# AntonXue/nn-sdp

Measured on NVIDIA B200. Metric: queries/sec (clique LMI blocks assembled: value * cliques_per_query), higher is better.
Workload: dtype f64

## Files before the change

### nn-sdp_b200/csrc/api.cu

```cuda
#include <math.h>
#include <stdarg.h>
#include <stdio.h>
#include <stdlib.h>
#include <string.h>

#include <algorithm>
#include <condition_variable>
#include <deque>
#include <functional>
#include <memory>
#include <mutex>
#include <thread>
#include <unordered_map>

#include <cuda.h>

#include "internal.h"

namespace nnsdp {

static thread_local std::string g_err;

void set_error(const char* fmt, ...) {
  char buf[1024];
// ... 748 lines not shown
  NN_TRY(b->xmax.ensure((size_t)sh.xtot * Q * 8));
  NN_TRY(b->acxmin.ensure((size_t)ac * Q * 8));
  NN_TRY(b->acxmax.ensure((size_t)ac * Q * 8));
  NN_TRY(b->smin_c.ensure((size_t)ac * Q * 8));
  NN_TRY(b->smax_c.ensure((size_t)ac * Q * 8));
  if (b->ring > 0) {
    const int npart = (int)((ac + PREP_THREADS - 1) / PREP_THREADS);
    NN_TRY(b->d11.ensure((size_t)ac * Q * 8));
    NN_TRY(b->Md.ensure((size_t)ac * Q * 8));
    NN_TRY(b->T0.ensure((size_t)ac * Q * 8));
    NN_TRY(b->Bt.ensure((size_t)ac * Q * 8 * std::max<int64_t>(beta, 1)));
    NN_TRY(b->u.ensure((size_t)ac * Q * 8));
    NN_TRY(b->aff.ensure((size_t)sh.Zdim * Q * 8));
    NN_TRY(b->part.ensure((size_t)npart * Q * 8));
    NN_TRY(b->act.ensure((size_t)ac * Q * 4));
    NN_TRY(b->cnt.ensure((size_t)sh.K * Q * 4));
    NN_TRY(b->Z11.ensure((size_t)sh.n_in() * sh.n_in() * Q * 8));
    NN_TRY(b->Z1K.ensure((size_t)sh.n_in() * sh.n[sh.K - 1] * Q * 8));
    NN_TRY(b->U.ensure((size_t)sh.n_out() * sh.n[sh.K - 1] * Q * 8));
    b->bd.npart = npart;
    const long long go = gram_layout(sh, &b->goff, &b->ldG);
    b->gram_per_query = go;
    NN_TRY(upload(b->d_goff, b->goff.data(), b->goff.size() * 8, b->st));
    NN_TRY(upload(b->d_ldG, b->ldG.data(), b->ldG.size() * 4, b->st));
    NN_TRY(b->gram.ensure((size_t)go * b->ring * 8));
    std::vector<CliqueRanges> mats;
    NN_TRY(format_mats(sh, beta, dense_Z, &mats));
    const char* noclass = getenv("NNSDP_NO_TILE_CLASSES");
    NN_TRY(build_plan(sh, beta, mats, b->packed || !(noclass && noclass[0] == '1'), &b->plan,
                      b->packed ? &b->lay : nullptr));
    b->mats_host = mats;
    for (const BandDev& j : b->plan.bands) b->band_max_m = std::max(b->band_max_m, j.m);
    b->nbands = (int)b->plan.bands.size();
    NN_TRY(upload(b->d_bands, b->plan.bands.data(), b->plan.bands.size() * sizeof(BandDev), b->st));
    if (!b->packed) NN_TRY(build_gather_plan(sh, beta, mats, b->plan, &b->gp));
    if (const char* e = getenv("NNSDP_DENSE_GATHER"))
      if (e[0] == '1') b->gp.usable = false;
    if (b->gp.usable) {
      NN_TRY(upload(b->d_thin_idx, b->gp.thin_idx.data(), b->gp.thin_idx.size() * 8, b->st));
      for (int i = 0; i < GATHER_STAGES; ++i)
        NN_CUDA(cudaEventCreateWithFlags(&b->ev_packed[i], cudaEventDisableTiming));
    }
    NN_TRY(upload(b->d_tiles, b->plan.tiles.data(), b->plan.tiles.size() * sizeof(TileDev), b->st));
    NN_TRY(upload(b->d_mats, b->plan.mats.data(), b->plan.mats.size() * sizeof(MatDev), b->st));
    NN_TRY(b->ringbuf.ensure((size_t)b->plan.per_query_doubles * b->ring * 8));
    b->slot_bulk.assign((size_t)b->ring * sh.K, 0);
    auto is_bulk = [&](const StripDev& d) {
      return !b->packed && d.rblk >= 1 && d.rblk <= sh.K - 1 &&
             (d.prog == PROG_SAME || (d.prog == PROG_DIAG && !b->plan.band_inline));
    };
    std::vector<StripDev> strips, bulk;
    std::vector<std::vector<StripDev>> per_blk(sh.K);
    b->pass_entries = 0;
    b->bulk_entries.assign(sh.K, 0);
    for (const StripDev& d : b->plan.strips) {
      if (d.prog == PROG_ZERO) continue;
      if (is_bulk(d)) {
        per_blk[d.rblk].push_back(d);
        b->bulk_entries[d.rblk] += (int64_t)d.nrows * d.ncols;
      } else {
        strips.push_back(d);
        b->pass_entries += (int64_t)d.nrows * d.ncols;
      }
    }
    b->bulk_begin.assign(sh.K + 1, 0);
    for (int blk = 0; blk < sh.K; ++blk) {
      b->bulk_begin[blk] = (int)bulk.size();
      bulk.insert(bulk.end(), per_blk[blk].begin(), per_blk[blk].end());
    }
    b->bulk_begin[sh.K] = (int)bulk.size();
    for (int i = b->plan.n_fill; i < (int)b->plan.tiles.size(); ++i)
      b->pass_entries += (int64_t)b->plan.tiles[i].nrows * b->plan.tiles[i].ncols;
    for (const BandDev& j : b->plan.bands)
      if (j.ld > 0) b->pass_entries += (int64_t)j.m * (2 * beta + 1) - beta * (beta + 1);
    NN_TRY(upload(b->d_strips, strips.data(), strips.size() * sizeof(StripDev), b->st));
    NN_TRY(upload(b->d_bulk, bulk.data(), bulk.size() * sizeof(StripDev), b->st));
    b->pd.strips = b->d_strips.as<StripDev>();
    b->pd.bulk = b->d_bulk.as<StripDev>();
    b->pd.n_strips = (int)strips.size();
    b->pd.tiles = b->d_tiles.as<TileDev>();
    b->pd.mats = b->d_mats.as<MatDev>();
    b->pd.panel_desc = nullptr;
    b->pd.n_panel = 0;
    {
      static const int panel_env = [] { const char* e = getenv("NNSDP_PANEL"); return e ? atoi(e) : 1; }();
      if (panel_env && !b->packed && !b->plan.panel.empty()) {
        std::vector<StripDev> panel;
        for (const StripDev& d : b->plan.panel)
          if (d.prog != PROG_ZERO && (d.prog == PROG_RC || d.prog == PROG_CR || !is_bulk(d))) panel.push_back(d);
        NN_TRY(upload(b->d_panel, panel.data(), panel.size() * sizeof(StripDev), b->st));
        b->pd.panel_desc = b->d_panel.as<StripDev>();
        b->pd.n_panel = (int)panel.size();
      }
    }
    b->pd.ntiles = (int)b->plan.tiles.size();
    b->pd.n_fill = b->plan.n_fill;
    b->pd.n_window = b->plan.n_window;
    b->pd.n_edge = b->plan.n_edge;
    b->pd.tile_rows = b->plan.tile_rows;
    b->pd.per_query = b->plan.per_query_doubles;
    b->pd.tmaps = nullptr;
    b->pd.tmap_ok = nullptr;
    if (b->plan.n_window > 0 && beta <= MAX_WINDOW_BETA) {
      typedef CUresult (*EncodeFn)(CUtensorMap*, CUtensorMapDataType, cuuint32_t, void*, const cuuint64_t*, const cuuint64_t*,
                                   const cuuint32_t*, const cuuint32_t*, CUtensorMapInterleave, CUtensorMapSwizzle,
                                   CUtensorMapL2promotion, CUtensorMapFloatOOBfill);
      void* fn = nullptr;
      cudaDriverEntryPointQueryResult qres;
      static const bool no_tma = [] { const char* e = getenv("NNSDP_NO_TMA"); return e && e[0] == '1'; }();
      if (!no_tma && cudaGetDriverEntryPoint("cuTensorMapEncodeTiled", &fn, cudaEnableDefault, &qres) == cudaSuccess && fn &&
          qres == cudaDriverEntryPointSuccess) {
        std::vector<CUtensorMap> maps(sh.K);
        std::vector<int> ok(sh.K, 0);
        bool any = false;
        for (int k = 0; k < sh.K; ++k) {
          if (sh.n[k + 1] % 2 != 0) continue;
          const cuuint64_t dims[2] = {(cuuint64_t)sh.n[k + 1], (cuuint64_t)sh.n[k]};
          const cuuint64_t strides[1] = {(cuuint64_t)sh.n[k + 1] * 8};
          const cuuint32_t box[2] = {(cuuint32_t)(128 + 2 * beta + 2), 32};
          const cuuint32_t estr[2] = {1, 1};
          const CUresult r = ((EncodeFn)fn)(&maps[k], CU_TENSOR_MAP_DATA_TYPE_FLOAT64, 2, b->nd->M[k].p, dims, strides, box, estr,
                                            CU_TENSOR_MAP_INTERLEAVE_NONE, CU_TENSOR_MAP_SWIZZLE_NONE,
                                            CU_TENSOR_MAP_L2_PROMOTION_L2_128B, CU_TENSOR_MAP_FLOAT_OOB_FILL_NONE);
          ok[k] = (r == CUDA_SUCCESS);
          any |= ok[k] != 0;
        }
        if (any) {
          static_assert(sizeof(CUtensorMap) == 128, "CUtensorMap is 128 bytes");
          NN_TRY(upload(b->d_tmaps, maps.data(), maps.size() * sizeof(CUtensorMap), b->st));
          NN_TRY(upload(b->d_tmap_ok, ok.data(), ok.size() * 4, b->st));
          NN_CUDA(cudaStreamSynchronize(b->st));
          b->pd.tmaps = b->d_tmaps.p;
          b->pd.tmap_ok = b->d_tmap_ok.as<int>();
        }
      } else {
        cudaGetLastError();
      }
    }
    b->pd.packed = b->plan.skip_absent ? 1 : 0;
    b->pd.band_inline = b->plan.band_inline ? 1 : 0;
    b->gd.scratch = b->gram.as<double>();
    b->gd.per_query = go;
    b->gd.goff = b->d_goff.as<long long>();
    b->gd.ldG = b->d_ldG.as<int>();
    b->gd.mirror = b->packed && b->plan.skip_absent ? 0 : 1;
  }
  NN_CUDA(cudaStreamSynchronize(b->st));
  guard.b = nullptr;
  *out = b;
  return NNSDP_OK;
}

int32_t nnsdp_batch_set_inputs(nnsdp_batch* b, int64_t Q, const nnsdp_query_inputs* in) {
  NN_CHECK(b && in, NNSDP_ERR_ARG, "NULL argument");
  NN_CHECK(Q >= 1 && Q <= b->Qcap, NNSDP_ERR_ARG, "Q = %lld outside [1, Qcap = %lld]", (long long)Q,
           (long long)b->Qcap);
  NN_CUDA(cudaSetDevice(b->dev));
  const Shape& sh = b->net->sh;
  const nnsdp_sizes& sz = b->sz;
  BatchDev& bd = b->bd;
  cudaStream_t st = b->st;
  b->have_inputs = false;
  b->bounds_done = b->prepared = false;
  b->Q = Q;
  bd.Q = (int)Q;
  bd.beta = (int)b->beta;
  bd.lamdim = sz.lamdim;
  bd.sdim = (int)sz.sdim;
  NN_TRY(upload_cols(b->x1min, in->x1min, in->x1min_stride, sz.n_in, Q, st, &bd.s_x1min, "x1min"));
  NN_TRY(upload_cols(b->x1max, in->x1max, in->x1max_stride, sz.n_in, Q, st, &bd.s_x1max, "x1max"));
  bd.x1min = b->x1min.as<double>();
  bd.x1max = b->x1max.as<double>();
  b->bounds_supplied = (in->ymin != nullptr);
  if (b->bounds_supplied) {
    NN_TRY(upload_cols(b->ymin, in->ymin, in->ymin_stride, sz.acdim, Q, st, &bd.s_ymin, "ymin"));
// ... 1721 lines not shown
```

### nn-sdp_b200/csrc/internal.h

```cpp
#pragma once

#include <cuda_runtime.h>
#include <stdint.h>

#include <string>
#include <vector>

#include "../../include/nnsdp_b200.h"

namespace nnsdp {

void set_error(const char* fmt, ...);
int32_t cuda_fail(cudaError_t e, const char* what, const char* file, int line);

#define NN_CUDA(call)                                                                \
  do {                                                                               \
    cudaError_t _e = (call);                                                         \
    if (_e != cudaSuccess) return ::nnsdp::cuda_fail(_e, #call, __FILE__, __LINE__); \
  } while (0)

#define NN_CHECK(cond, code, ...)      \
  do {                                 \
    if (!(cond)) {                     \
      ::nnsdp::set_error(__VA_ARGS__); \
// ... 41 lines not shown
int32_t make_cliques_host(const Shape& sh, int64_t beta, CliqueInfoHost* out);
int64_t lambda_dim(int64_t acdim, int64_t beta);
long long gram_layout(const Shape& sh, std::vector<long long>* goff, std::vector<int>* ldG);
int32_t fill_sizes(const Shape& sh, int64_t beta, nnsdp_sizes* out);

enum TileFlags : uint32_t {
  TF_AFF = 1u << 0,
  TF_SAME = 1u << 1,
  TF_1K = 1u << 2,
  TF_RC = 1u << 3,
  TF_CR = 1u << 4,
  TF_BAND = 1u << 5,
  TF_ALL = 0x3Fu,
  TF_UNIFORM = 1u << 8,
};

enum TileProg : int32_t {
  PROG_ZERO = 0, PROG_SAME = 1, PROG_RC = 2, PROG_CR = 3, PROG_MIXED = 4, PROG_GENERAL = 5,
  PROG_DIAG = 6, PROG_AFF = 7,
};

struct TileDev {
  int32_t mat;
  int32_t row0, nrows;
  int32_t col0, ncols;
  int32_t grow0;
  int32_t gcol0;
  uint32_t flags;
  int32_t rblk, cblk;
  int32_t prog;
};

struct alignas(16) StripDev {
  long long out_off;
  long long goff;
  int32_t ld, row0, nrows, col0;
  int32_t ncols, grow0, gcol0, prog;
  int32_t rblk, rl0, cl0, ldG;
};
static_assert(sizeof(StripDev) == 64, "StripDev must be 64 bytes");

struct MatDev {
  int64_t out_off;
  int32_t n;
  int32_t ld;
};

enum PackedKind : int32_t { PK_WINDOW = 1, PK_DIAG = 2, PK_BAND = 3, PK_RECT = 4 };
struct PackedCell {
  int32_t kind, blk;
  int64_t grow0, gcol0;
  int64_t nrows, ncols;
  int64_t offset;
  int32_t always;
};
struct PackedLayout {
  std::vector<PackedCell> cells;
  int64_t record_doubles = 0;
  int64_t always_doubles = 0;
  int64_t always_entries = 0;
  std::vector<int32_t> diag_cell;
  std::vector<int64_t> diag_entries;
};
struct BandDev {
  long long out_off;
  long long band_off;
  int ld, row0, col0;
  int g0, m, blk;
  int optional;
  int upper_only;
};

struct PlanHost {
  std::vector<StripDev> strips;
  std::vector<TileDev> tiles;
  std::vector<MatDev> mats;
  int64_t per_query_doubles = 0;
  int tile_rows = 0, tile_cols = 0;
  std::vector<BandDev> bands;
  bool band_inline = true;
  int n_fill = 0, n_window = 0, n_edge = 0;
  bool skip_absent = false;
  std::vector<StripDev> panel;
};

enum GatherKind : int32_t { GK_NONE = 0, GK_ALWAYS = 1, GK_GRAM = 2, GK_S22 = 3 };
constexpr int GATHER_MIN_RECT = 256;

struct GatherCell {
  int32_t row0, nrows;
  int32_t kind, blk;
  int32_t pure_zero;
  int32_t ncols_hint, col0_hint;
};
struct GatherColSeg {
  int32_t mat, col0, ncols;
  std::vector<GatherCell> cells;
};
struct GatherPlan {
  bool usable = false;
  std::vector<GatherColSeg> colsegs;
  std::vector<int32_t> colseg_begin;
  std::vector<int64_t> thin_idx;
  std::vector<int64_t> thin_begin;
  int64_t dense_always_doubles = 0;
};

int32_t build_plan(const Shape& sh, int64_t beta, const std::vector<CliqueRanges>& mats,
                   bool classify, PlanHost* plan, PackedLayout* packed = nullptr);
void unpack_record(const Shape& sh, int64_t beta, const PackedLayout& lay, const std::vector<CliqueRanges>& mats,
                   const double* record, const uint8_t* present, double* out);
int32_t build_gather_plan(const Shape& sh, int64_t beta, const std::vector<CliqueRanges>& mats,
                          const PlanHost& plan, GatherPlan* gp);

struct NetDev {
  int K, n_in, n_out, Zdim, acdim, xtot;
  const int* n;
  const int* off;
  const int* xoff;
  const int* blk_of;
  const double* const* M;
  const double* const* Wt;
  const int* ldT;
  const double* bias_all;
};

struct BatchDev {
  int Q, beta;
  int out_kind, has_s22, has_s12;
  int sdim;
  long long lamdim;
  const double* x1min;   long long s_x1min;
  const double* x1max;   long long s_x1max;
  const double* ymin;    long long s_ymin;
  const double* ymax;    long long s_ymax;
  const double* smin;    long long s_smin;
  const double* smax;    long long s_smax;
  const double* gin;     long long s_gin;
  const double* gbnd;    long long s_gbnd;
  const double* gsec;    long long s_gsec;
  const double* outS;    long long s_outS;
  const double* outvec;  long long s_outvec;
  const double* outinvP; long long s_outinvP;
  const double* gout;    long long s_gout;
  double* d11;
  double* Md;
  double* T0;
  double* Bt;
  double* u;
  double* aff;
  double* part;
  int npart;
  int* act;
  int* cnt;
  double* Z11;
  double* Z1K;
  double* U;
};

struct GramDev {
  double* scratch;
  long long per_query;
  const long long* goff;
  const int* ldG;
  int mirror;
};

struct PlanDev {
  const StripDev* strips;
  const StripDev* bulk;
  int n_strips;
  const TileDev* tiles;
  const MatDev* mats;
  const StripDev* panel_desc;
  int n_panel;
  int ntiles;
  int n_fill, n_window, n_edge;
  int tile_rows;
  long long per_query;
  const void* tmaps;
  const int* tmap_ok;
  int packed;
  int band_inline;
};

int ibp_layer_launch(const double* Mk, int n_out_k, int n_in_k, const double* xin_min,
                     const double* xin_max, long long x_stride, double* xout_min, double* xout_max,
                     double* acx_min, double* acx_max, long long acx_stride, int Q, int relu,
                     int write_x, int* flag_bad, cudaStream_t st);
int affine_layer_launch(const double* Wt, int ldT, int n_rows, int n_neurons, const double* u,
                        long long u_stride, double* aff, long long aff_stride, int Q,
                        cudaStream_t st);
int affine_all_launch(const NetDev& nd, int K, int max_rows, const double* u, long long u_stride, double* aff,
                      long long aff_stride, int Q, cudaStream_t st);
int ibp_all_launch(const NetDev& nd, int max_out, const double* x1min, long long s_min, const double* x1max,
                   long long s_max, double* xmin, double* xmax, long long x_stride, double* acxmin, double* acxmax,
                   double* smin, double* smax, long long acx_stride, int Q, int* flag_bad, cudaStream_t st);
int dgemm_dmma_launch(const double* A, int lda, int M, int K, const double* B, long long ldb, double* C, long long ldc,
                      int N, int accumulate, cudaStream_t st);
int ibp_dmma_launch(const double* Mk, int n_out_k, int n_in_k, const double* xin_min, const double* xin_max,
                    long long x_stride, double* xout_min, double* xout_max, double* acx_min, double* acx_max,
                    long long acx_stride, int Q, int relu, int write_x, int* flag_bad, cudaStream_t st);
int dgemm_dmma_affine_layers_launch(const NetDev& nd, int b0, int nb, int max_rows, const double* u, long long u_stride,
                                    double* aff, long long aff_stride, int Q, cudaStream_t st);
int ibp_chain_launch(const NetDev& nd, int max_w, const double* x1min, long long s_min, const double* x1max,
                     long long s_max, double* xmin, double* xmax, long long x_stride, double* acxmin, double* acxmax,
                     double* smin, double* smax, long long acx_stride, int Q, int* flag_bad, cudaStream_t st);
int launch_sector_minmax(long long n, const double* acxmin, const double* acxmax, double* smin,
                         double* smax, cudaStream_t st);
int launch_place_x1(const double* x1min, long long s_min, const double* x1max, long long s_max,
                    double* xmin, double* xmax, long long xtot, int n_in, int Q, cudaStream_t st);
int launch_transpose_w(const double* Mk, int n_out_k, int n_in_k, double* Wt, int ldT,
                       cudaStream_t st);
int launch_prep(const NetDev& net, const BatchDev& b, int* err_flag, cudaStream_t st);
int launch_gram(const NetDev& net, const BatchDev& b, const GramDev& g, int max_n, int q0, const int* pairs,
                int npairs, cudaStream_t st);
struct BulkItem {
  int32_t slot, first, count;
};
constexpr int BULK_PER_LAUNCH = 512;
struct BulkSel {
  int32_t n;
  BulkItem item[BULK_PER_LAUNCH];
};
int launch_emit(const NetDev& net, const BatchDev& b, const GramDev& g, const PlanDev& plan,
                int q0, int nq, double* out, cudaStream_t st, int which, const BulkItem* sel, int nsel);

struct AffineDev {
  long long nvar, var_out, var_bnd, var_sec;
  long long acdim, lamdim, beta;
  int out_kind;
  const double *x1min, *x1max, *ymin, *ymax, *smin, *smax;
  long long s_x1min, s_x1max, s_ymin, s_ymax, s_smin, s_smax;
  const long long* col_ptr;
  const int* lo;
};
int launch_affine_count(const NetDev& net, const AffineDev& A, long long* counts, cudaStream_t st);
int launch_affine_fill(const NetDev& net, const AffineDev& A, const long long* offs, long long* ent,
                       long long* var, double* val, cudaStream_t st);
int launch_affine_z0(const NetDev& net, const BatchDev& b, const AffineDev& A, long long nent, int Q, double* z0,
                     cudaStream_t st);
int launch_affine_csc_count(const NetDev& net, const AffineDev& A, const long long* first, long long ngroups,
                            long long* counts, cudaStream_t st);
int launch_affine_csc_fill(const NetDev& net, const AffineDev& A, const long long* first, long long ngroups,
                           const long long* offs, long long* ent, double* val, cudaStream_t st);
long long scan_scratch_len(long long n);
int launch_scan_exclusive(long long* x, long long n, long long* sums, cudaStream_t st);
int launch_affine_group_starts(const long long* offs, long long nvar, long long ngroups, long long* starts,
                               cudaStream_t st);

int launch_eig_init(double* v, int Zdim, int Qc, int q_first, cudaStream_t st);
int launch_eig_mid(const NetDev& net, const BatchDev& b, int q_first, int Qc, const double* x,
                   const double* t, double* s1, double* y, cudaStream_t st);
int launch_eig_io(const NetDev& net, const BatchDev& b, int q_first, int Qc, const double* x, double* y,
                  cudaStream_t st);
int launch_eig_multidot(const double* V, const double* w, int n, int Qc, int nv, double* c, int c_ld,
                        cudaStream_t st);
int launch_eig_project(const double* V, double* w, int n, int Qc, int nv, const double* c, int c_ld,
// ... 47 lines not shown
```

### nn-sdp_b200/csrc/kernels_emit.cu

```cuda
#include <stdlib.h>

#include <algorithm>

#include "internal.h"

namespace nnsdp {

namespace {

constexpr int ETHREADS = 256;
constexpr int SLOT_GROUP = 8;
constexpr int FAST_TR = 128, FAST_TC = 32, FAST_NCOL = 16;
constexpr int MAX_TAPS = 2 * MAX_FAST_BETA + 1;
constexpr int MAX_TC = 32;

struct QView {
  const double* Md;
  const double* T0;
  const double* Bt;
  const double* gbnd;
  const double* aff;
  const double* Z11;
  const double* Z1K;
  const double* U;
// ... 427 lines not shown
  const bool copy = Br <= K - 2 && b.cnt[(long long)q * K + Br] > 0;
  const bool s22 = Br == K - 1 && b.has_s22;
  if (plan.packed && !copy && !s22) return;
  const double* WK = net.M[K - 1];
  const double* U = b.U + (long long)q * net.n_out * net.n[K - 1];
  const double* G = g.scratch + (long long)slot * g.per_query + goff + rl0;
  if (BAND_INLINE && prog == PROG_DIAG) {
    const int beta = b.beta;
    const long long acdim = net.acdim;
    const int jr_base = grow0 - net.n_in - row0, jc0 = gcol0 - net.n_in;
    const double* T0 = b.T0 + (long long)q * acdim;
    const double* Bt = b.Bt + (long long)q * beta * acdim;
    const double* gbnd = b.gbnd + q * b.s_gbnd;
    const double* Gc = G + (long long)(cl0 + cg) * ldG;
    const long long gstep = (long long)ncg * ldG;
    for (int c = cg; c < ncols; c += ncg, col += cstep, Gc += gstep) {
      const int jc = jc0 + c;
      int r = row0 - (int)(((size_t)(col + row0) >> 3) & 3) + tr;
      for (; r < row_end; r += TR) {
        if (r < row0) continue;
        double v = copy ? Gc[r] : (s22 ? s22_entry(WK, U, net.n_out, rl0 + r, cl0 + c) : 0.0);
        const int d = jr_base + r - jc;
        if (d >= -beta && d <= beta) {
          v = 0.0 + v;
          v += 0.0;
          v = __dadd_rn(v, band_term(T0, gbnd, Bt, acdim, jc + d, jc));
        }
        col[r] = v;
      }
    }
  } else if (copy) {
    const double* Gc = G + (long long)(cl0 + cg) * ldG;
    const long long gstep = (long long)ncg * ldG;
    for (int c = cg; c < ncols; c += ncg, col += cstep, Gc += gstep) {
      int r = row0 - (int)(((size_t)(col + row0) >> 3) & 3) + tr;
      if (r >= row0 && r < row_end) col[r] = Gc[r];
      for (r += TR; r < row_end; r += TR) col[r] = Gc[r];
    }
  } else if (s22) {
    NNSDP_STRIP_LOOP(s22_entry(WK, U, net.n_out, rl0 + r, cl0 + c))
  } else {
    NNSDP_STRIP_LOOP(0.0)
  }
#undef NNSDP_STRIP_LOOP
}

template <bool BAND_INLINE>
__global__ void __launch_bounds__(ETHREADS, NNSDP_FILL_MINB)
emit_fill_kernel(NetDev net, BatchDev b, GramDev g, PlanDev plan, int q0, int nq,
                 double* __restrict__ out) {
  fill_strip<BAND_INLINE>(net, b, g, plan, plan.strips + blockIdx.x, blockIdx.y, q0, out);
}

template <bool BAND_INLINE>
__global__ void __launch_bounds__(ETHREADS, NNSDP_FILL_MINB)
emit_fill_kernel(NetDev net, BatchDev b, GramDev g, PlanDev plan, int q0, BulkSel sel, double* __restrict__ out) {
  const BulkItem it = sel.item[blockIdx.y];
  if ((int)blockIdx.x >= it.count) return;
  fill_strip<BAND_INLINE>(net, b, g, plan, plan.bulk + it.first + blockIdx.x, it.slot, q0, out);
}

template <int BETA>
__global__ void __launch_bounds__(ETHREADS, 4)
emit_window_kernel(NetDev net, BatchDev b, PlanDev plan, int tile0, int q0, int nq, int group, int group_major,
                   double* __restrict__ out) {
  constexpr int RC_DOUBLES = SLOT_GROUP * (BETA + 1) * (FAST_TC + BETA + 1), CR_DOUBLES = FAST_TC * CR_LDW(BETA);
  __shared__ __align__(128) double smem[RC_DOUBLES > CR_DOUBLES ? RC_DOUBLES : CR_DOUBLES];
  __shared__ __align__(8) unsigned long long mbar;
  const int ngroups = (nq + group - 1) / group;
  const int ti = group_major ? blockIdx.x % plan.n_window : blockIdx.x / ngroups;
  const int gi = group_major ? blockIdx.x / plan.n_window : blockIdx.x % ngroups;
  const TileDev t = plan.tiles[tile0 + ti];
  const MatDev mat = plan.mats[t.mat];
  const int slot0 = gi * group;
  const int nslots = min(group, nq - slot0);
  if (t.prog == PROG_RC) {
    if (t.ncols == FAST_TC) emit_rc<BETA, true>(net, b, plan, t, mat, q0, slot0, nslots, out, smem);
    else emit_rc<BETA, false>(net, b, plan, t, mat, q0, slot0, nslots, out, smem);
  } else {
    emit_cr<BETA>(net, b, plan, t, mat, q0, slot0, nslots, out, smem, &mbar);
  }
}

template <int BETA>
__global__ void __launch_bounds__(ETHREADS, 4)
emit_panel_kernel(NetDev net, BatchDev b, GramDev g, PlanDev plan, int q0, int nq, int group, double* __restrict__ out) {
  constexpr int RC_DOUBLES = SLOT_GROUP * (BETA + 1) * (FAST_TC + BETA + 1), CR_DOUBLES = FAST_TC * CR_LDW(BETA);
  __shared__ __align__(128) double smem[RC_DOUBLES > CR_DOUBLES ? RC_DOUBLES : CR_DOUBLES];
  __shared__ __align__(8) unsigned long long mbar;
  const int batch = group >> 8;
  group &= 255;
  const int gb = batch / group;
  const int per_batch = plan.n_panel * gb;
  const int sb = blockIdx.x / per_batch, rem = blockIdx.x - sb * per_batch;
  const int slot_lo = sb * batch, slot_hi = min(nq, slot_lo + batch);
  const int item = rem / gb, g0 = rem - item * gb;
  const StripDev* desc = plan.panel_desc + item;
  const int4* dp = reinterpret_cast<const int4*>(desc);
  const int4 d2 = __ldg(dp + 2);
  if (d2.w != PROG_RC && d2.w != PROG_CR) {
    for (int slot = slot_lo + g0; slot < slot_hi; slot += gb) fill_strip<false>(net, b, g, plan, desc, slot, q0, out);
    return;
  }
  const int4 d0 = __ldg(dp), d1 = __ldg(dp + 1), d3 = __ldg(dp + 3);
  TileDev t;
  t.mat = 0;
  t.row0 = d1.y, t.nrows = d1.z, t.col0 = d1.w, t.ncols = d2.x, t.grow0 = d2.y, t.gcol0 = d2.z, t.prog = d2.w;
  t.rblk = d3.x, t.cblk = d3.y, t.flags = (uint32_t)d3.z;
  MatDev mat;
  mat.out_off = ((long long)(unsigned)d0.x) | ((long long)d0.y << 32);
  mat.ld = d1.x;
  mat.n = d3.w;
  const int slot0 = slot_lo + g0 * group;
  const int nslots = min(group, slot_hi - slot0);
  if (nslots <= 0) return;
  if (t.prog == PROG_RC) {
    if (t.ncols == FAST_TC) emit_rc<BETA, true>(net, b, plan, t, mat, q0, slot0, nslots, out, smem);
    else emit_rc<BETA, false>(net, b, plan, t, mat, q0, slot0, nslots, out, smem);
  } else {
    emit_cr<BETA>(net, b, plan, t, mat, q0, slot0, nslots, out, smem, &mbar);
  }
}

__global__ void __launch_bounds__(ETHREADS, 4)
emit_edge_kernel(NetDev net, BatchDev b, GramDev g, PlanDev plan, int tile0, int q0, int nq,
                 int group, double* __restrict__ out) {
  __shared__ double smem[MAX_TC * MAX_TAPS + 128 * MAX_TAPS];
  const TileDev t = plan.tiles[tile0 + blockIdx.x];
  const MatDev mat = plan.mats[t.mat];
  const int slot0 = blockIdx.y * group;
  const int nslots = min(group, nq - slot0);
  int TR = 1;
  while (TR < t.nrows) TR <<= 1;
  if (TR > ETHREADS) TR = ETHREADS;
  const int tr = threadIdx.x % TR, cg = threadIdx.x / TR, ncg = ETHREADS / TR;
  const long long tile_off = mat.out_off + (t.row0 + tr) + (long long)t.col0 * mat.ld;
  const bool uniform = (t.flags & TF_UNIFORM) != 0 && t.nrows * t.ncols > 512;
  if (uniform) {
    for (int s = 0; s < nslots; ++s) {
      const QView v = make_view(net, b, g, q0 + slot0 + s, slot0 + s);
      double* o = out + (long long)(slot0 + s) * plan.per_query + tile_off;
      emit_mixed(net, b, g, t, mat, v, o, tr, cg, ncg, smem);
    }
    return;
  }
  int TC = 1;
  while (TC < t.ncols && TC < ncg) TC <<= 1;
  const int per = TR * TC;
  const int spar = ETHREADS / per;
  const int sub = threadIdx.x / per, cg2 = (threadIdx.x % per) / TR;
  for (int s = sub; s < nslots; s += spar) {
    const QView v = make_view(net, b, g, q0 + slot0 + s, slot0 + s);
    double* o = out + (long long)(slot0 + s) * plan.per_query + tile_off;
    emit_general(net, b, g, t, mat, v, o, tr, cg2, TC);
  }
}

}

namespace {
__device__ __forceinline__ void band_entry(const NetDev& net, const BatchDev& b, const GramDev& g, const BandDev& bd,
                                           long long per_query, int q0, int slot, int idx, double* __restrict__ out) {
  const int q = q0 + slot, K = net.K, beta = b.beta, nt = 2 * beta + 1;
  if (idx >= bd.m * nt) return;
  const int i = idx / nt, t = idx - i * nt - beta, c = i + t;
  if (bd.upper_only && t < 0) return;
  double* o = out + (long long)slot * per_query;
  if (c < 0 || c >= bd.m) {
    if (bd.band_off >= 0 && t >= 0) o[bd.band_off + t + (long long)(beta + 1) * i] = 0.0;
    return;
  }
  const int Br = bd.blk, n0 = net.n_in;
  const long long acdim = net.acdim;
  const int rl = bd.g0 - net.off[Br] + i, cl = rl + t;
  const int jr = bd.g0 + i - n0, jc = jr + t;
  const bool copy = Br <= K - 2 && b.cnt[(long long)q * K + Br] > 0;
  const bool s22 = Br == K - 1 && b.has_s22;
  double val = 0.0;
  if (copy) val += g.scratch[(long long)slot * g.per_query + g.goff[Br] + rl + (long long)cl * g.ldG[Br]];
  if (s22) val += s22_entry(net.M[K - 1], b.U + (long long)q * net.n_out * net.n[K - 1], net.n_out, rl, cl);
  val += 0.0;
  val = __dadd_rn(val, band_term(b.T0 + (long long)q * acdim, b.gbnd + q * b.s_gbnd, b.Bt + (long long)q * beta * acdim,
                                 acdim, jr, jc));
  if (bd.ld > 0 && (!bd.optional || copy || s22)) o[bd.out_off + (bd.row0 + i) + (long long)(bd.col0 + c) * bd.ld] = val;
  if (bd.band_off >= 0 && t >= 0) o[bd.band_off + t + (long long)(beta + 1) * i] = val;
}

__global__ void __launch_bounds__(ETHREADS)
emit_band_kernel(NetDev net, BatchDev b, GramDev g, const BandDev* __restrict__ bands, long long per_query, int q0,
                 int nq, int spc, double* __restrict__ out) {
  const BandDev bd = bands[blockIdx.y];
  const int idx = blockIdx.x * ETHREADS + threadIdx.x;
  for (int slot = blockIdx.z * spc; slot < min(nq, (blockIdx.z + 1) * spc); ++slot)
    band_entry(net, b, g, bd, per_query, q0, slot, idx, out);
}
}

int launch_emit_band(const NetDev& net, const BatchDev& b, const GramDev& g, const BandDev* bands, int nbands,
                     int max_m, long long per_query, int q0, int nq, double* out, cudaStream_t st) {
  if (nbands <= 0 || nq <= 0 || max_m <= 0) return 0;
  const int nx = (max_m * (2 * b.beta + 1) + ETHREADS - 1) / ETHREADS;
  static const int spc_env = [] { const char* e = getenv("NNSDP_BAND_GROUP"); return e ? atoi(e) : 0; }();
  const int spc = spc_env > 0 ? spc_env : (nq >= 16 ? 4 : 1);
  emit_band_kernel<<<dim3(nx, nbands, (nq + spc - 1) / spc), ETHREADS, 0, st>>>(net, b, g, bands, per_query, q0, nq, spc, out);
  return 1;
}

namespace {
__global__ void pack_thin_kernel(const double* __restrict__ ring, long long per_query,
                                 const long long* __restrict__ idx, long long nthin,
                                 double* __restrict__ packed, int nq) {
  const long long total = nthin * nq;
  for (long long i = blockIdx.x * (long long)blockDim.x + threadIdx.x; i < total;
       i += (long long)gridDim.x * blockDim.x) {
    const long long s = i / nthin, k = i - s * nthin;
    packed[i] = ring[s * per_query + idx[k]];
  }
}
}

int launch_pack_thin(const double* ring, long long per_query, const long long* idx, long long nthin,
                     double* packed, int nq, cudaStream_t st) {
  if (nthin <= 0 || nq <= 0) return 0;
  long long blocks = (nthin * nq + 255) / 256;
  if (blocks > 148 * 16) blocks = 148 * 16;
  pack_thin_kernel<<<(int)blocks, 256, 0, st>>>(ring, per_query, idx, nthin, packed, nq);
  return 1;
}

static int launch_bulk(const NetDev& net, const BatchDev& b, const GramDev& g, const PlanDev& plan, int q0,
                       const BulkItem* sel, int nsel, double* out, cudaStream_t st) {
  int launches = 0;
  for (int i0 = 0; i0 < nsel; i0 += BULK_PER_LAUNCH) {
    BulkSel s;
    s.n = std::min(BULK_PER_LAUNCH, nsel - i0);
    int most = 0;
    for (int i = 0; i < s.n; ++i) {
      s.item[i] = sel[i0 + i];
      most = std::max(most, s.item[i].count);
    }
    if (most == 0) continue;
    const dim3 grid((unsigned)most, (unsigned)s.n);
    if (plan.band_inline) emit_fill_kernel<true><<<grid, ETHREADS, 0, st>>>(net, b, g, plan, q0, s, out);
    else emit_fill_kernel<false><<<grid, ETHREADS, 0, st>>>(net, b, g, plan, q0, s, out);
    ++launches;
  }
  return launches;
}

int launch_emit(const NetDev& net, const BatchDev& b, const GramDev& g, const PlanDev& plan,
                int q0, int nq, double* out, cudaStream_t st, int which, const BulkItem* sel, int nsel) {
  if (nq <= 0) return 0;
  static const int wgroup = [] { const char* e = getenv("NNSDP_WINDOW_GROUP"); int v = e ? atoi(e) : 4; return v < 1 ? 1 : (v > SLOT_GROUP ? SLOT_GROUP : v); }();
  static const int egroup_env = [] { const char* e = getenv("NNSDP_EDGE_GROUP"); int v = e ? atoi(e) : 0; return v < 0 ? 0 : (v > SLOT_GROUP ? SLOT_GROUP : v); }();
  const int egroup = egroup_env > 0 ? egroup_env : (nq >= 64 ? SLOT_GROUP : (nq >= 16 ? 4 : 1));
  int launches = 0;
  if (plan.n_panel > 0 && b.beta <= MAX_WINDOW_BETA) {
    if (which < 0 || which == 0) {
      static const int pgroup = [] { const char* e = getenv("NNSDP_PANEL_GROUP"); int v = e ? atoi(e) : 2; return v < 1 ? 1 : (v > SLOT_GROUP ? SLOT_GROUP : v); }();
      static const int pbatch_env = [] { const char* e = getenv("NNSDP_PANEL_BATCH"); return e ? atoi(e) : 8; }();
      int pbatch = std::max(pgroup, (pbatch_env / pgroup) * pgroup);
      if (pbatch > 255) pbatch = (255 / pgroup) * pgroup;
      const int nbatches = (nq + pbatch - 1) / pbatch;
      const dim3 grid((unsigned)plan.n_panel * (pbatch / pgroup) * nbatches);
      switch (b.beta) {
        case 0: emit_panel_kernel<0><<<grid, ETHREADS, 0, st>>>(net, b, g, plan, q0, nq, pgroup | (pbatch << 8), out); break;
        case 1: emit_panel_kernel<1><<<grid, ETHREADS, 0, st>>>(net, b, g, plan, q0, nq, pgroup | (pbatch << 8), out); break;
        case 2: emit_panel_kernel<2><<<grid, ETHREADS, 0, st>>>(net, b, g, plan, q0, nq, pgroup | (pbatch << 8), out); break;
        case 3: emit_panel_kernel<3><<<grid, ETHREADS, 0, st>>>(net, b, g, plan, q0, nq, pgroup | (pbatch << 8), out); break;
        default: emit_panel_kernel<4><<<grid, ETHREADS, 0, st>>>(net, b, g, plan, q0, nq, pgroup | (pbatch << 8), out); break;
      }
      ++launches;
    }
  } else {
  if (plan.n_strips > 0 && (which < 0 || which == 0)) {
    if (plan.band_inline) emit_fill_kernel<true><<<dim3(plan.n_strips, nq), ETHREADS, 0, st>>>(net, b, g, plan, q0, nq, out);
    else emit_fill_kernel<false><<<dim3(plan.n_strips, nq), ETHREADS, 0, st>>>(net, b, g, plan, q0, nq, out);
    ++launches;
  }
  if (plan.n_window > 0 && (which < 0 || which == 1)) {
    const dim3 grid(plan.n_window * ((nq + wgroup - 1) / wgroup));
    const int t0 = plan.n_fill;
    static const int gm_env = [] { const char* e = getenv("NNSDP_WINDOW_GROUP_MAJOR"); return e ? atoi(e) : -1; }();
    const int gm = gm_env >= 0 ? gm_env : plan.band_inline;
    switch (b.beta) {
      case 0: emit_window_kernel<0><<<grid, ETHREADS, 0, st>>>(net, b, plan, t0, q0, nq, wgroup, gm, out); break;
      case 1: emit_window_kernel<1><<<grid, ETHREADS, 0, st>>>(net, b, plan, t0, q0, nq, wgroup, gm, out); break;
      case 2: emit_window_kernel<2><<<grid, ETHREADS, 0, st>>>(net, b, plan, t0, q0, nq, wgroup, gm, out); break;
      case 3: emit_window_kernel<3><<<grid, ETHREADS, 0, st>>>(net, b, plan, t0, q0, nq, wgroup, gm, out); break;
      case 4: emit_window_kernel<4><<<grid, ETHREADS, 0, st>>>(net, b, plan, t0, q0, nq, wgroup, gm, out); break;
      default: return -1;
    }
    ++launches;
  }
  }
  if (which < 0 || which == 0) launches += launch_bulk(net, b, g, plan, q0, sel, nsel, out, st);
  if (plan.n_edge > 0 && (which < 0 || which == 2)) {
    emit_edge_kernel<<<dim3(plan.n_edge, (nq + egroup - 1) / egroup), ETHREADS, 0, st>>>(
        net, b, g, plan, plan.n_fill + plan.n_window, q0, nq, egroup, out);
    ++launches;
  }
  return launches;
}

}
```

### nn-sdp_b200/csrc/plan.cpp

```cpp
#include <stdint.h>
#include <stdlib.h>

#include <algorithm>

#include "internal.h"
#include <atomic>
#include <cstring>
#include <thread>

namespace nnsdp {

int64_t lambda_dim(int64_t acdim, int64_t beta) {
  int64_t s = 0;
  for (int64_t t = acdim - beta; t <= acdim; ++t) s += t;
  return s;
}

long long gram_layout(const Shape& sh, std::vector<long long>* goff, std::vector<int>* ldG) {
  goff->assign(sh.K, 0);
  ldG->assign(sh.K, 0);
  long long go = 0;
  for (int blk = 0; blk <= sh.K - 2; ++blk) {
    (*ldG)[blk] = (int)(((sh.n[blk] + 15) / 16) * 16);
    (*goff)[blk] = go;
// ... 487 lines not shown
      }
      NN_CHECK(cell >= 0, NNSDP_ERR_STATE, "packed plan: a tile lies in no cell");
      const PackedCell& c = L.cells[cell];
      t.mat = cell;
      t.row0 = (int32_t)(t.grow0 - c.grow0);
      t.col0 = (int32_t)(t.gcol0 - c.gcol0);
      if (c.kind == PK_DIAG) L.diag_entries[c.blk] += (int64_t)t.nrows * t.ncols;
      else L.always_entries += (int64_t)t.nrows * t.ncols;
    }
    for (const PackedCell& c : band) L.always_entries += c.nrows * c.ncols;
    plan->per_query_doubles = L.record_doubles;
  }
  std::stable_sort(plan->tiles.begin(), plan->tiles.end(),
                   [&](const TileDev& x, const TileDev& y) { return cls(x) < cls(y); });
  {
    std::vector<long long> goff;
    std::vector<int> ldG;
    gram_layout(sh, &goff, &ldG);
    plan->strips.clear();
    for (const TileDev& t : plan->tiles) {
      if (cls(t) != 0) break;
      StripDev d{};
      d.out_off = plan->mats[t.mat].out_off;
      d.ld = plan->mats[t.mat].ld;
      d.row0 = t.row0; d.nrows = t.nrows; d.col0 = t.col0; d.ncols = t.ncols;
      d.grow0 = t.grow0; d.gcol0 = t.gcol0; d.prog = t.prog; d.rblk = t.rblk;
      if ((t.prog == PROG_SAME || t.prog == PROG_DIAG) && t.rblk >= 0) {
        d.rl0 = (int32_t)(t.grow0 - sh.off[t.rblk] - t.row0);
        d.cl0 = (int32_t)(t.gcol0 - sh.off[t.rblk]);
        if (t.rblk <= K - 2) {
          d.goff = goff[t.rblk];
          d.ldG = ldG[t.rblk];
        }
      }
      plan->strips.push_back(d);
    }
  }
  {
    plan->bands.clear();
    struct Box { int64_t lo = INT64_MAX, hi = -1, l0 = 0; bool band = false; };
    std::vector<std::vector<Box>> box(plan->mats.size(), std::vector<Box>(K));
    int64_t widest = 0;
    for (const TileDev& t : plan->tiles) {
      if (cls(t) != 0 || !(t.prog == PROG_SAME || t.prog == PROG_DIAG) || t.rblk < 1 || t.rblk != t.cblk) continue;
      Box& bx = box[t.mat][t.rblk];
      const int64_t lo = std::min<int64_t>(t.grow0, t.gcol0);
      if (lo < bx.lo) {
        bx.lo = lo;
        bx.l0 = (t.grow0 <= t.gcol0) ? t.row0 : t.col0;
      }
      bx.hi = std::max<int64_t>(bx.hi, std::max<int64_t>(t.grow0 + t.nrows, t.gcol0 + t.ncols) - 1);
      bx.band |= (t.prog == PROG_DIAG);
      widest = std::max<int64_t>(widest, bx.hi - bx.lo + 1);
    }
    plan->band_inline = widest < 256;
    for (size_t m = 0; m < plan->mats.size(); ++m)
      for (int blk = 1; blk < K; ++blk) {
        const Box& bx = box[m][blk];
        if (bx.hi < bx.lo || !bx.band) continue;
        BandDev j{};
        j.out_off = plan->mats[m].out_off;
        j.band_off = -1;
        j.ld = plan->band_inline ? 0 : plan->mats[m].ld;
        j.row0 = j.col0 = (int)bx.l0;
        j.g0 = (int)bx.lo;
        j.m = (int)(bx.hi - bx.lo + 1);
        j.blk = blk;
        if (packed) {
          const PackedCell& c = packed->cells[m];
          j.optional = (c.kind == PK_DIAG);
          j.upper_only = 1;
          for (const PackedCell& bc : packed->cells)
            if (bc.kind == PK_BAND && bc.blk == blk) j.band_off = bc.offset;
        }
        if (j.ld > 0 || j.band_off >= 0) plan->bands.push_back(j);
      }
  }
  plan->n_fill = plan->n_window = plan->n_edge = 0;
  for (const TileDev& t : plan->tiles) {
    const int c = cls(t);
    (c == 0 ? plan->n_fill : c == 1 ? plan->n_window : plan->n_edge)++;
  }
  plan->panel.clear();
  if (!packed && !plan->band_inline && plan->n_window > 0 && beta <= MAX_WINDOW_BETA) {
    struct Key { long long off; int panel, row0, col0, code; };
    std::vector<Key> keys;
    keys.reserve((size_t)plan->n_fill + plan->n_window);
    for (int i = 0; i < plan->n_fill; ++i) {
      const StripDev& d = plan->strips[i];
      keys.push_back({d.out_off, d.col0 / 32, d.row0, d.col0, i});
    }
    for (int i = 0; i < plan->n_window; ++i) {
      const TileDev& t = plan->tiles[plan->n_fill + i];
      keys.push_back({plan->mats[t.mat].out_off, t.col0 / 32, t.row0, t.col0, ~i});
    }
    std::stable_sort(keys.begin(), keys.end(), [](const Key& x, const Key& y) {
      if (x.off != y.off) return x.off < y.off;
      if (x.panel != y.panel) return x.panel < y.panel;
      if (x.col0 != y.col0) return x.col0 < y.col0;
      return x.row0 < y.row0;
    });
    plan->panel.resize(keys.size());
    for (size_t i = 0; i < keys.size(); ++i) {
      const int code = keys[i].code;
      if (code >= 0) {
        plan->panel[i] = plan->strips[code];
        continue;
      }
      const TileDev& t = plan->tiles[plan->n_fill + ~code];
      const MatDev& m = plan->mats[t.mat];
      StripDev d{};
      d.out_off = m.out_off;
      d.ld = m.ld;
      d.row0 = t.row0; d.nrows = t.nrows; d.col0 = t.col0; d.ncols = t.ncols;
      d.grow0 = t.grow0; d.gcol0 = t.gcol0; d.prog = t.prog;
      d.rblk = t.rblk; d.rl0 = t.cblk; d.cl0 = (int32_t)t.flags; d.ldG = m.n;
      plan->panel[i] = d;
    }
  }
  return NNSDP_OK;
}


static void unpack_one(int64_t beta, const PackedLayout& lay, const CliqueRanges& ck, const double* record,
                       const uint8_t* present, double* o) {
  const int64_t n = ck.size();
  std::memset(o, 0, (size_t)n * n * sizeof(double));
  constexpr int64_t TB = 64;
  auto copy_rect = [&](const PackedCell& c) {
    const double* src = record + c.offset;
    int64_t rbase = 0;
    for (int sr = 0; sr < ck.nseg; rbase += ck.hi[sr] - ck.lo[sr] + 1, ++sr) {
      const int64_t r0 = std::max(c.grow0, ck.lo[sr]), r1 = std::min(c.grow0 + c.nrows - 1, ck.hi[sr]);
      if (r0 > r1) continue;
      int64_t cbase = 0;
      for (int sc = 0; sc < ck.nseg; cbase += ck.hi[sc] - ck.lo[sc] + 1, ++sc) {
        const int64_t c0 = std::max(c.gcol0, ck.lo[sc]), c1 = std::min(c.gcol0 + c.ncols - 1, ck.hi[sc]);
        if (c0 > c1 || r0 > c1) continue;
        const int64_t lr_of = rbase - ck.lo[sr], lc_of = cbase - ck.lo[sc];
        for (int64_t gcb = std::max(c0, r0); gcb <= c1; gcb += TB) {
          const int64_t gce = std::min(gcb + TB - 1, c1);
          for (int64_t grb = r0; grb <= std::min(r1, gce); grb += TB) {
            const int64_t gre = std::min(grb + TB - 1, r1);
            for (int64_t gc = gcb; gc <= gce; ++gc) {
              const int64_t rhi = std::min(gre, gc);
              if (grb > rhi) continue;
              const double* col = src + (gc - c.gcol0) * c.nrows - c.grow0;
              std::memcpy(o + (lr_of + grb) + (lc_of + gc) * n, col + grb, (size_t)(rhi - grb + 1) * sizeof(double));
            }
            for (int64_t gr = grb; gr <= gre; ++gr) {
              const int64_t glo = std::max(gcb, gr);
              if (glo > gce) continue;
              double* dst = o + (lr_of + gr) * n + lc_of;
              const double* s0 = src - c.grow0 + gr - c.gcol0 * c.nrows;
              for (int64_t gc = glo; gc <= gce; ++gc) dst[gc] = s0[gc * c.nrows];
            }
          }
        }
      }
    }
  };
  auto local = [&](int64_t g) -> int64_t {
    int64_t base = 0;
    for (int s = 0; s < ck.nseg; base += ck.hi[s] - ck.lo[s] + 1, ++s)
      if (g >= ck.lo[s] && g <= ck.hi[s]) return base + g - ck.lo[s];
    return -1;
  };
  for (int pass : {PK_DIAG, PK_WINDOW, PK_BAND, PK_RECT})
    for (size_t i = 0; i < lay.cells.size(); ++i) {
      const PackedCell& c = lay.cells[i];
      if (c.kind != pass || !present[i]) continue;
      if (c.kind != PK_BAND) {
        copy_rect(c);
        continue;
      }
      const double* src = record + c.offset;
      for (int64_t j = 0; j < c.ncols; ++j) {
        const int64_t lr = local(c.grow0 + j);
        if (lr < 0) continue;
        for (int64_t t = 0; t <= beta && j + t < c.ncols; ++t) {
          const int64_t lc = local(c.grow0 + j + t);
          if (lc < 0) continue;
          const double v = src[t + (beta + 1) * j];
          o[lr + lc * n] = v;
          o[lc + lr * n] = v;
        }
      }
    }
}

void unpack_record(const Shape& sh, int64_t beta, const PackedLayout& lay, const std::vector<CliqueRanges>& mats,
                   const double* record, const uint8_t* present, double* out) {
  (void)sh;
  std::vector<int64_t> off(mats.size() + 1, 0);
  for (size_t m = 0; m < mats.size(); ++m) off[m + 1] = off[m] + mats[m].size() * mats[m].size();
  int nthreads = 1;
  if (mats.size() > 1 && off.back() >= (int64_t(1) << 20)) {
    const char* e = getenv("NNSDP_HOST_THREADS");
    const unsigned hw = std::thread::hardware_concurrency();
    nthreads = e ? atoi(e) : (int)std::min<unsigned>(hw ? hw : 1, 16);
    nthreads = std::max(1, std::min<int>(nthreads, (int)mats.size()));
// ... 106 lines not shown
```

Measured before the change: 9274.

## Fold edge tiles into the panel kernel to drop the separate edge launch

Edge tiles (mixed/general programs) are added to a second sorted panel descriptor list and handled inside the panel kernel via a shared emit_edge_tile helper, so the separate emit_edge_kernel launch is skipped when folding is on. It is on by default and can be turned off with NNSDP_PANEL_FOLD=0. The aim is to save a kernel launch and to let edge work overlap with window and fill work in the same grid, keeping writes ordered by output panel. In exchange, one panel block now processes all slots of its batch for an edge tile, which can cause load imbalance. The panel kernel also gains a template variant, which may raise compile time and code size.

```diff
diff --git a/nn-sdp_b200/csrc/api.cu b/nn-sdp_b200/csrc/api.cu
--- a/nn-sdp_b200/csrc/api.cu
+++ b/nn-sdp_b200/csrc/api.cu
@@ -854,15 +854,19 @@
     b->pd.mats = b->d_mats.as<MatDev>();
     b->pd.panel_desc = nullptr;
     b->pd.n_panel = 0;
+    b->pd.fold = 0;
     {
       static const int panel_env = [] { const char* e = getenv("NNSDP_PANEL"); return e ? atoi(e) : 1; }();
       if (panel_env && !b->packed && !b->plan.panel.empty()) {
+        const char* fold_env = getenv("NNSDP_PANEL_FOLD");
+        const bool fold = !(fold_env && atoi(fold_env) == 0);
         std::vector<StripDev> panel;
-        for (const StripDev& d : b->plan.panel)
+        for (const StripDev& d : fold ? b->plan.panel_fold : b->plan.panel)
           if (d.prog != PROG_ZERO && (d.prog == PROG_RC || d.prog == PROG_CR || !is_bulk(d))) panel.push_back(d);
         NN_TRY(upload(b->d_panel, panel.data(), panel.size() * sizeof(StripDev), b->st));
         b->pd.panel_desc = b->d_panel.as<StripDev>();
         b->pd.n_panel = (int)panel.size();
+        b->pd.fold = fold ? 1 : 0;
       }
     }
     b->pd.ntiles = (int)b->plan.tiles.size();
diff --git a/nn-sdp_b200/csrc/internal.h b/nn-sdp_b200/csrc/internal.h
--- a/nn-sdp_b200/csrc/internal.h
+++ b/nn-sdp_b200/csrc/internal.h
@@ -147,6 +147,7 @@
   int n_fill = 0, n_window = 0, n_edge = 0;
   bool skip_absent = false;
   std::vector<StripDev> panel;
+  std::vector<StripDev> panel_fold;
 };
 
 enum GatherKind : int32_t { GK_NONE = 0, GK_ALWAYS = 1, GK_GRAM = 2, GK_S22 = 3 };
@@ -239,6 +240,7 @@
   const MatDev* mats;
   const StripDev* panel_desc;
   int n_panel;
+  int fold;
   int ntiles;
   int n_fill, n_window, n_edge;
   int tile_rows;
diff --git a/nn-sdp_b200/csrc/kernels_emit.cu b/nn-sdp_b200/csrc/kernels_emit.cu
--- a/nn-sdp_b200/csrc/kernels_emit.cu
+++ b/nn-sdp_b200/csrc/kernels_emit.cu
@@ -533,11 +533,54 @@
   }
 }
 
-template <int BETA>
+constexpr int EDGE_DOUBLES = MAX_TC * MAX_TAPS + 128 * MAX_TAPS;
+
+__device__ __forceinline__ void emit_edge_tile(const NetDev& net, const BatchDev& b, const GramDev& g,
+                                               const PlanDev& plan, const TileDev& t, const MatDev& mat, int q0,
+                                               int slot0, int nslots, double* __restrict__ out, double* smem) {
+  int TR = 1;
+  while (TR < t.nrows) TR <<= 1;
+  if (TR > ETHREADS) TR = ETHREADS;
+  const int tr = threadIdx.x % TR, cg = threadIdx.x / TR, ncg = ETHREADS / TR;
+  const long long tile_off = mat.out_off + (t.row0 + tr) + (long long)t.col0 * mat.ld;
+  const bool uniform = (t.flags & TF_UNIFORM) != 0 && t.nrows * t.ncols > 512;
+  if (uniform) {
+    for (int s = 0; s < nslots; ++s) {
+      const QView v = make_view(net, b, g, q0 + slot0 + s, slot0 + s);
+      double* o = out + (long long)(slot0 + s) * plan.per_query + tile_off;
+      emit_mixed(net, b, g, t, mat, v, o, tr, cg, ncg, smem);
+    }
+    return;
+  }
+  int TC = 1;
+  while (TC < t.ncols && TC < ncg) TC <<= 1;
+  const int per = TR * TC;
+  const int spar = ETHREADS / per;
+  const int sub = threadIdx.x / per, cg2 = (threadIdx.x % per) / TR;
+  for (int s = sub; s < nslots; s += spar) {
+    const QView v = make_view(net, b, g, q0 + slot0 + s, slot0 + s);
+    double* o = out + (long long)(slot0 + s) * plan.per_query + tile_off;
+    emit_general(net, b, g, t, mat, v, o, tr, cg2, TC);
+  }
+}
+
+__global__ void __launch_bounds__(ETHREADS, 4)
+emit_edge_kernel(NetDev net, BatchDev b, GramDev g, PlanDev plan, int tile0, int q0, int nq,
+                 int group, double* __restrict__ out) {
+  __shared__ double smem[EDGE_DOUBLES];
+  const TileDev t = plan.tiles[tile0 + blockIdx.x];
+  const MatDev mat = plan.mats[t.mat];
+  const int slot0 = blockIdx.y * group;
+  emit_edge_tile(net, b, g, plan, t, mat, q0, slot0, min(group, nq - slot0), out, smem);
+}
+
+template <int BETA, bool FOLD>
 __global__ void __launch_bounds__(ETHREADS, 4)
 emit_panel_kernel(NetDev net, BatchDev b, GramDev g, PlanDev plan, int q0, int nq, int group, double* __restrict__ out) {
   constexpr int RC_DOUBLES = SLOT_GROUP * (BETA + 1) * (FAST_TC + BETA + 1), CR_DOUBLES = FAST_TC * CR_LDW(BETA);
-  __shared__ __align__(128) double smem[RC_DOUBLES > CR_DOUBLES ? RC_DOUBLES : CR_DOUBLES];
+  constexpr int WIN_DOUBLES = RC_DOUBLES > CR_DOUBLES ? RC_DOUBLES : CR_DOUBLES;
+  static_assert(WIN_DOUBLES >= EDGE_DOUBLES, "the edge tiles stage their band coefficients in the same buffer");
+  __shared__ __align__(128) double smem[WIN_DOUBLES];
   __shared__ __align__(8) unsigned long long mbar;
   const int batch = group >> 8;
   group &= 255;
@@ -549,10 +592,11 @@
   const StripDev* desc = plan.panel_desc + item;
   const int4* dp = reinterpret_cast<const int4*>(desc);
   const int4 d2 = __ldg(dp + 2);
-  if (d2.w != PROG_RC && d2.w != PROG_CR) {
+  if (d2.w != PROG_RC && d2.w != PROG_CR && !(FOLD && (d2.w == PROG_MIXED || d2.w == PROG_GENERAL))) {
     for (int slot = slot_lo + g0; slot < slot_hi; slot += gb) fill_strip<false>(net, b, g, plan, desc, slot, q0, out);
     return;
   }
+  if (FOLD && (d2.w == PROG_MIXED || d2.w == PROG_GENERAL) && g0 != 0) return;
   const int4 d0 = __ldg(dp), d1 = __ldg(dp + 1), d3 = __ldg(dp + 3);
   TileDev t;
   t.mat = 0;
@@ -562,6 +606,10 @@
   mat.out_off = ((long long)(unsigned)d0.x) | ((long long)d0.y << 32);
   mat.ld = d1.x;
   mat.n = d3.w;
+  if (FOLD && t.prog != PROG_RC && t.prog != PROG_CR) {
+    emit_edge_tile(net, b, g, plan, t, mat, q0, slot_lo, slot_hi - slot_lo, out, smem);
+    return;
+  }
   const int slot0 = slot_lo + g0 * group;
   const int nslots = min(group, slot_hi - slot0);
   if (nslots <= 0) return;
@@ -570,40 +618,6 @@
     else emit_rc<BETA, false>(net, b, plan, t, mat, q0, slot0, nslots, out, smem);
   } else {
     emit_cr<BETA>(net, b, plan, t, mat, q0, slot0, nslots, out, smem, &mbar);
-  }
-}
-
-__global__ void __launch_bounds__(ETHREADS, 4)
-emit_edge_kernel(NetDev net, BatchDev b, GramDev g, PlanDev plan, int tile0, int q0, int nq,
-                 int group, double* __restrict__ out) {
-  __shared__ double smem[MAX_TC * MAX_TAPS + 128 * MAX_TAPS];
-  const TileDev t = plan.tiles[tile0 + blockIdx.x];
-  const MatDev mat = plan.mats[t.mat];
-  const int slot0 = blockIdx.y * group;
-  const int nslots = min(group, nq - slot0);
-  int TR = 1;
-  while (TR < t.nrows) TR <<= 1;
-  if (TR > ETHREADS) TR = ETHREADS;
-  const int tr = threadIdx.x % TR, cg = threadIdx.x / TR, ncg = ETHREADS / TR;
-  const long long tile_off = mat.out_off + (t.row0 + tr) + (long long)t.col0 * mat.ld;
-  const bool uniform = (t.flags & TF_UNIFORM) != 0 && t.nrows * t.ncols > 512;
-  if (uniform) {
-    for (int s = 0; s < nslots; ++s) {
-      const QView v = make_view(net, b, g, q0 + slot0 + s, slot0 + s);
-      double* o = out + (long long)(slot0 + s) * plan.per_query + tile_off;
-      emit_mixed(net, b, g, t, mat, v, o, tr, cg, ncg, smem);
-    }
-    return;
-  }
-  int TC = 1;
-  while (TC < t.ncols && TC < ncg) TC <<= 1;
-  const int per = TR * TC;
-  const int spar = ETHREADS / per;
-  const int sub = threadIdx.x / per, cg2 = (threadIdx.x % per) / TR;
-  for (int s = sub; s < nslots; s += spar) {
-    const QView v = make_view(net, b, g, q0 + slot0 + s, slot0 + s);
-    double* o = out + (long long)(slot0 + s) * plan.per_query + tile_off;
-    emit_general(net, b, g, t, mat, v, o, tr, cg2, TC);
   }
 }
 
@@ -714,13 +728,18 @@
       if (pbatch > 255) pbatch = (255 / pgroup) * pgroup;
       const int nbatches = (nq + pbatch - 1) / pbatch;
       const dim3 grid((unsigned)plan.n_panel * (pbatch / pgroup) * nbatches);
+      const int gp = pgroup | (pbatch << 8);
+#define NNSDP_PANEL_LAUNCH(B)                                                                                  \
+  if (plan.fold) emit_panel_kernel<B, true><<<grid, ETHREADS, 0, st>>>(net, b, g, plan, q0, nq, gp, out);      \
+  else emit_panel_kernel<B, false><<<grid, ETHREADS, 0, st>>>(net, b, g, plan, q0, nq, gp, out);
       switch (b.beta) {
-        case 0: emit_panel_kernel<0><<<grid, ETHREADS, 0, st>>>(net, b, g, plan, q0, nq, pgroup | (pbatch << 8), out); break;
-        case 1: emit_panel_kernel<1><<<grid, ETHREADS, 0, st>>>(net, b, g, plan, q0, nq, pgroup | (pbatch << 8), out); break;
-        case 2: emit_panel_kernel<2><<<grid, ETHREADS, 0, st>>>(net, b, g, plan, q0, nq, pgroup | (pbatch << 8), out); break;
-        case 3: emit_panel_kernel<3><<<grid, ETHREADS, 0, st>>>(net, b, g, plan, q0, nq, pgroup | (pbatch << 8), out); break;
-        default: emit_panel_kernel<4><<<grid, ETHREADS, 0, st>>>(net, b, g, plan, q0, nq, pgroup | (pbatch << 8), out); break;
-      }
+        case 0: NNSDP_PANEL_LAUNCH(0) break;
+        case 1: NNSDP_PANEL_LAUNCH(1) break;
+        case 2: NNSDP_PANEL_LAUNCH(2) break;
+        case 3: NNSDP_PANEL_LAUNCH(3) break;
+        default: NNSDP_PANEL_LAUNCH(4) break;
+      }
+#undef NNSDP_PANEL_LAUNCH
       ++launches;
     }
   } else {
@@ -746,7 +765,7 @@
   }
   }
   if (which < 0 || which == 0) launches += launch_bulk(net, b, g, plan, q0, sel, nsel, out, st);
-  if (plan.n_edge > 0 && (which < 0 || which == 2)) {
+  if (!plan.fold && plan.n_edge > 0 && (which < 0 || which == 2)) {
     emit_edge_kernel<<<dim3(plan.n_edge, (nq + egroup - 1) / egroup), ETHREADS, 0, st>>>(
         net, b, g, plan, plan.n_fill + plan.n_window, q0, nq, egroup, out);
     ++launches;
diff --git a/nn-sdp_b200/csrc/plan.cpp b/nn-sdp_b200/csrc/plan.cpp
--- a/nn-sdp_b200/csrc/plan.cpp
+++ b/nn-sdp_b200/csrc/plan.cpp
@@ -593,32 +593,22 @@
     (c == 0 ? plan->n_fill : c == 1 ? plan->n_window : plan->n_edge)++;
   }
   plan->panel.clear();
+  plan->panel_fold.clear();
   if (!packed && !plan->band_inline && plan->n_window > 0 && beta <= MAX_WINDOW_BETA) {
-    struct Key { long long off; int panel, row0, col0, code; };
+    struct Key { long long off; int panel, row0, col0; StripDev d; };
     std::vector<Key> keys;
-    keys.reserve((size_t)plan->n_fill + plan->n_window);
-    for (int i = 0; i < plan->n_fill; ++i) {
-      const StripDev& d = plan->strips[i];
-      keys.push_back({d.out_off, d.col0 / 32, d.row0, d.col0, i});
-    }
-    for (int i = 0; i < plan->n_window; ++i) {
-      const TileDev& t = plan->tiles[plan->n_fill + i];
-      keys.push_back({plan->mats[t.mat].out_off, t.col0 / 32, t.row0, t.col0, ~i});
-    }
-    std::stable_sort(keys.begin(), keys.end(), [](const Key& x, const Key& y) {
-      if (x.off != y.off) return x.off < y.off;
-      if (x.panel != y.panel) return x.panel < y.panel;
-      if (x.col0 != y.col0) return x.col0 < y.col0;
-      return x.row0 < y.row0;
-    });
-    plan->panel.resize(keys.size());
-    for (size_t i = 0; i < keys.size(); ++i) {
-      const int code = keys[i].code;
-      if (code >= 0) {
-        plan->panel[i] = plan->strips[code];
-        continue;
-      }
-      const TileDev& t = plan->tiles[plan->n_fill + ~code];
+    auto sorted = [](std::vector<Key> k) {
+      std::stable_sort(k.begin(), k.end(), [](const Key& x, const Key& y) {
+        if (x.off != y.off) return x.off < y.off;
+        if (x.panel != y.panel) return x.panel < y.panel;
+        if (x.col0 != y.col0) return x.col0 < y.col0;
+        return x.row0 < y.row0;
+      });
+      std::vector<StripDev> v(k.size());
+      for (size_t i = 0; i < k.size(); ++i) v[i] = k[i].d;
+      return v;
+    };
+    auto add_tile = [&](const TileDev& t) {
       const MatDev& m = plan->mats[t.mat];
       StripDev d{};
       d.out_off = m.out_off;
@@ -626,8 +616,16 @@
       d.row0 = t.row0; d.nrows = t.nrows; d.col0 = t.col0; d.ncols = t.ncols;
       d.grow0 = t.grow0; d.gcol0 = t.gcol0; d.prog = t.prog;
       d.rblk = t.rblk; d.rl0 = t.cblk; d.cl0 = (int32_t)t.flags; d.ldG = m.n;
-      plan->panel[i] = d;
-    }
+      keys.push_back({d.out_off, d.col0 / 32, d.row0, d.col0, d});
+    };
+    for (int i = 0; i < plan->n_fill; ++i) {
+      const StripDev& d = plan->strips[i];
+      keys.push_back({d.out_off, d.col0 / 32, d.row0, d.col0, d});
+    }
+    for (int i = 0; i < plan->n_window; ++i) add_tile(plan->tiles[plan->n_fill + i]);
+    plan->panel = sorted(keys);
+    for (int i = 0; i < plan->n_edge; ++i) add_tile(plan->tiles[plan->n_fill + plan->n_window + i]);
+    plan->panel_fold = sorted(keys);
   }
   return NNSDP_OK;
 }
```

Result: faster. 9574, median of 6 (+3.2%).
